# segeschecho/OpenEKFMonoSLAM

Measured on AMD Instinct MI355X. Metric: EKF updates/s (frames/s) at N features, higher is better.
Workload: dtype f32 storage; i8 MFMA with exact i32 sums (downdate) + f64 (B, S, state)

## Files before the change

include/ekf_test_hooks.h:

```cpp
#ifndef EKF_TEST_HOOKS_H
#define EKF_TEST_HOOKS_H

#include "ekf_engine.h"

#ifdef __cplusplus
extern "C" {
#endif

int ekf_debug_stall_next_sweep(EkfEngine *e);
int ekf_debug_stall_sweep_after(EkfEngine *e, int skip);
int ekf_debug_plane0_pieces(EkfEngine *e, int *nonzero, int *total);
int ekf_debug_dense_products(EkfEngine *e, int on);

#ifdef __cplusplus
}
#endif
#endif
```

openekfmonoslam_amd/csrc/engine.cpp:

```cpp
#include "engine.h"
#include "../../include/ekf_test_hooks.h"

#include <cmath>
#include <cstdio>
#include <algorithm>
#include <atomic>
#include <cstdlib>
#include <chrono>
#include <cstring>
#include <mutex>
#include <new>

#include <dlfcn.h>
#include <rccl/rccl.h>

using namespace ekf;

namespace ekf {
void launch_partition(EkfEngine *e, const EkfMatch *src, int M, const uint8_t *flags, EkfMatch *dst1, EkfMatch *dst0,
                      int *cnt1, bool map_update = false, const uint8_t *d_kdesc = nullptr, int *d_idx0 = nullptr,
                      int publish_seq = 0, bool rescue = false);
void launch_outlier_idx(EkfEngine *e, const EkfMatch *src, int M, int *idx);
}

// ... 1336 lines not shown
            e->pu_log.emplace_back(e->pu_m[i], ms);
        }
        (void)hipEventDestroy(e->pu_events[i].first);
        (void)hipEventDestroy(e->pu_events[i].second);
    }
    e->pu_events.clear();
    e->pu_work.clear();
    e->pu_m.clear();
    for (size_t i = 0; i < e->sw_events.size(); ++i) {
        float ms = 0.f;
        if (hipEventElapsedTime(&ms, e->sw_events[i].first, e->sw_events[i].second) == hipSuccess) {
            const double m = std::abs(e->sw_m[i]);
            e->sweep_ms += ms;
            e->sweep_panels += ((long long)m + NB - 1) / NB;
            e->sweep_launches += i < e->sw_launch.size() ? e->sw_launch[i] : 0;
            e->sweep_updates += 1;
            e->sweep_flops_f64 += m * m * m / 3.0;
            if (e->sw_m[i] > 0) e->sweep_flops_b += m * m * (double)e->n;
        }
        (void)hipEventDestroy(e->sw_events[i].first);
        (void)hipEventDestroy(e->sw_events[i].second);
    }
    e->sw_events.clear();
    e->sw_launch.clear();
    e->sw_m.clear();
}

struct StageTimer {
    EkfEngine *e;
    std::vector<hipEvent_t> evs;
    explicit StageTimer(EkfEngine *eng) : e(eng) {}
    ~StageTimer()
    {
        for (auto ev : evs) (void)hipEventDestroy(ev);
    }
    void mark()
    {
        if (!e->timing) return;
        hipEvent_t ev;
        if (hipEventCreate(&ev) != hipSuccess) return;
        (void)hipEventRecord(ev, e->stream);
        evs.push_back(ev);
    }
    void finish()
    {
        if (!e->timing || evs.size() < 7) return;
        (void)hipStreamSynchronize(e->stream);
        double *dst[6] = {&e->times.prediction_ms, &e->times.matching_ms, &e->times.ransac_ms,
                          &e->times.update_li_ms,  &e->times.rescue_ms,   &e->times.update_hi_ms};
        for (int i = 0; i < 6; ++i) {
            float ms = 0.f;
            if (hipEventElapsedTime(&ms, evs[i], evs[i + 1]) == hipSuccess) *dst[i] += ms;
        }
        for (auto ev : evs) (void)hipEventDestroy(ev);
        evs.clear();
        e->times.steps += 1;
        harvest_pu_events(e);
    }
};

static int match_ncc_dev(EkfEngine *e, int *n_matches);

static int detect_step_keypoints(EkfEngine *e);

static int step_dev(EkfEngine *e, const EkfKeypoint *d_kps, const uint8_t *d_desc, int n_kp, EkfStepInfo *info,
                    bool use_ncc = false, bool detect = false)
{
    const bool dev_counts = !use_ncc && !detect && !e->img.valid && !e->keep_step_preds && e->shard_world == 1;
    const bool lean = e->shard_world > 1;
    int *cnt = e->d.counts;
    EkfStepInfo li;
    std::memset(&li, 0, sizeof(li));
    int status = EKF_OK, rc;
    const int retries0 = e->sweep_retries;
    if (!dev_counts && e->err_unread) {
        if ((rc = read_counts(e))) return rc;
        if ((rc = recover_failed_update(e, &status))) return rc;
    }
    bool restarted = false;
restart:
    StageTimer tm(e);
    tm.mark();
    int np = 0;
    if (dev_counts) {
        const bool deferred = launch_predict_with_features(e, e->N);
        launch_hp_rows(e, e->d.plist, e->N, true, cnt + CNT_NPRED, deferred);
    } else {
        launch_predict(e);
        if ((rc = predict_measurements_dev(e, nullptr, e->N, &np, true, lean))) return rc;
    }
    tm.mark();
    int M = 0;
    if (dev_counts) {
        launch_match(e, d_kps, d_desc, e->N, n_kp, cnt + CNT_NPRED, true);
    } else {
        if (detect && (rc = detect_step_keypoints(e))) return rc;
        if (lean) rc = match_sharded_dev(e, use_ncc, d_kps, d_desc, n_kp, &M);
        else rc = use_ncc ? match_ncc_dev(e, &M) : match_dev(e, d_kps, d_desc, n_kp, &M, detect ? cnt + CNT_KP_FOUND : nullptr);
        if (rc) return rc;
    }
    tm.mark();
    if (dev_counts) {
        const int batch = e->cfg.ransac_batch;
        const int seq_r = next_publish_seq(e);
        launch_ransac_batch(e, e->N, 0, batch, cnt + CNT_NMATCH, seq_r);
        if ((rc = wait_counts(e, seq_r))) return rc;
        if (e->h_counts[CNT_ERR] && !restarted) {
            if ((rc = recover_failed_update(e, &status))) return rc;
            restarted = true;
            goto restart;
        }
        np = e->n_pred = e->h_counts[CNT_NPRED];
        M = e->h_counts[CNT_NMATCH];
        for (int h0 = batch, nb = batch * RANSAC_WIDE_FACTOR; !e->h_counts[CNT_RS_DONE] && h0 < M; h0 += nb) {
            launch_ransac_batch(e, M, h0, nb);
            if ((rc = read_counts(e))) return rc;
        }
    } else if (M > 0 && (rc = ransac_dev(e, M, lean))) {
        return rc;
    }
    li.n_predicted = np;
    li.n_matches = M;
    int ni = 0, no = 0;
    if (M > 0) {
        li.n_hypotheses = e->h_counts[CNT_RS_NEXT];
        ni = e->h_counts[CNT_RS_BEST];
        no = M - ni;
        launch_partition(e, e->d.matches, M, e->d.best_flags, e->d.msel, e->d.mout, nullptr, true, d_desc, e->d.work_idx);
    }
    li.n_inliers = ni;
    li.n_outliers = no;
    tm.mark();
    if ((rc = update_dev(e, ni, true, lean))) return rc;
    tm.mark();
    int nr = 0;
    if (no > 0) {
        int nop = 0;
        for (int attempt = 0; attempt < 2; ++attempt) {
            if (dev_counts) {
                launch_predict_features(e, e->d.work_idx, no, false);
                launch_hp_rows(e, e->d.plist_sub, no, false, cnt + CNT_NPRED_SUB);
                const int seq_p = next_publish_seq(e);
                launch_partition(e, e->d.mout, no, e->d.mask, e->d.msel, nullptr, cnt + CNT_NRESC, true, d_desc, nullptr, seq_p, true);
                rc = wait_counts(e, seq_p);
            } else {
                rc = predict_measurements_dev(e, e->d.work_idx, no, &nop, false, lean);
            }
            if (rc) return rc;
            if (!e->h_counts[CNT_ERR]) break;
            if ((rc = recover_failed_update(e, &status))) return rc;
        }
        if (dev_counts) {
            nr = e->h_counts[CNT_NRESC];
        } else if (nop > 0) {
            launch_rescue(e, e->d.mout, no);
            launch_partition(e, e->d.mout, no, e->d.mask, e->d.msel, nullptr, cnt + CNT_NRESC, true, d_desc);
            if ((rc = read_counts(e))) return rc;
            nr = e->h_counts[CNT_NRESC];
        }
    }
    li.n_rescued = nr;
    tm.mark();
    if ((rc = update_dev(e, nr, true, lean))) return rc;
    tm.mark();
    if (dev_counts && e->async_errors) {
        e->err_unread = true;
    } else {
        if ((rc = read_counts(e))) return rc;
        if (detect) {
            e->step_kp_detected = e->h_counts[CNT_KP_FOUND];
            e->step_kp_kept = std::min(e->step_kp_detected, e->kcap);
        }
        if ((rc = recover_failed_update(e, &status))) return rc;
    }
    tm.finish();
    li.status = status;
    li.n_sweep_retries = e->sweep_retries - retries0;
    if (info) *info = li;
    return status;
}

int ekf_set_async_errors(EkfEngine *e, int on)
{
    if (!e) return EKF_ERR_INVALID_ARG;
    e->async_errors = on != 0;
    return EKF_OK;
}

// ... 446 lines not shown
        launch_ncc_pyramid_on(e, e->stream2, e->img.px2, e->img.seq + (size_t)(frame + 1) * frame_bytes, e->img.seq_stride,
                              e->img.seq_channels);
        HIPCHK(hipEventRecord(e->ev_prefetch, e->stream2));
        e->img.prefetched = frame + 1;
    }
    return EKF_OK;
}

int ekf_select_staged_image(EkfEngine *e, int frame)
{
    if (!e) return EKF_ERR_INVALID_ARG;
    HIPCHK(hipSetDevice(e->device));
    int rc = staged_pyramid(e, frame);
    return rc ? rc : check_async(e);
}

int ekf_step_staged_image(EkfEngine *e, int frame, EkfStepInfo *info)
{
    if (!e) return EKF_ERR_INVALID_ARG;
    HIPCHK(hipSetDevice(e->device));
    int rc = staged_pyramid(e, frame);
    if (rc) return rc;
    return step_image_dev(e, info);
}

int ekf_timing_enable(EkfEngine *e, int on)
{
    if (!e) return EKF_ERR_INVALID_ARG;
    e->timing = on != 0;
    return EKF_OK;
}

int ekf_timing_reset(EkfEngine *e)
{
    if (!e) return EKF_ERR_INVALID_ARG;
    (void)hipStreamSynchronize(e->stream);
    harvest_pu_events(e);
    e->pu_log.clear();
    std::memset(&e->times, 0, sizeof(e->times));
    e->sweep_ms = e->sweep_flops_f64 = e->sweep_flops_b = 0.0;
    e->sweep_panels = e->sweep_updates = e->sweep_launches = 0;
    e->slice_ms = 0.0;
    return EKF_OK;
}

int ekf_timing_get(EkfEngine *e, EkfStageTimes *out)
{
    if (!e || !out) return EKF_ERR_INVALID_ARG;
    (void)hipStreamSynchronize(e->stream);
    harvest_pu_events(e);
    *out = e->times;
    return EKF_OK;
}

int ekf_timing_sweep(EkfEngine *e, double *kernel_ms, int64_t *panels, int64_t *updates, double *flops_fp64, double *flops_b)
{
    if (!e) return EKF_ERR_INVALID_ARG;
    (void)hipStreamSynchronize(e->stream);
    harvest_pu_events(e);
    if (kernel_ms) *kernel_ms = e->sweep_ms;
    if (panels) *panels = e->sweep_panels;
    if (updates) *updates = e->sweep_updates;
    if (flops_fp64) *flops_fp64 = e->sweep_flops_f64;
    if (flops_b) *flops_b = e->sweep_flops_b;
    return EKF_OK;
}

int ekf_get_sweep_retries(const EkfEngine *e) { return e ? e->sweep_retries : 0; }

int ekf_debug_stall_next_sweep(EkfEngine *e)
{
    if (!e) return EKF_ERR_INVALID_ARG;
    e->ps_fault = 1;
    return EKF_OK;
}

int ekf_debug_dense_products(EkfEngine *e, int on)
{
    if (!e) return EKF_ERR_INVALID_ARG;
    e->px_dense = on != 0;
    return EKF_OK;
}

int ekf_debug_plane0_pieces(EkfEngine *e, int *nonzero, int *total)
{
    if (!e || !nonzero || !total || !e->d.Bz) return EKF_ERR_INVALID_ARG;
    HIPCHK(hipSetDevice(e->device));
    HIPCHK(hipStreamSynchronize(e->stream));
    const int cbs = (e->n + 31) / 32, groups = (2 * e->last_update_M + 15) / 16;
    std::vector<uint8_t> row((size_t)e->bz_stride);
    int nz = 0;
    for (int c = 0; c < cbs; ++c) {
        HIPCHK(hipMemcpy(row.data(), e->d.Bz + (size_t)c * e->bz_stride, (size_t)groups, hipMemcpyDeviceToHost));
        for (int k = 0; k < groups; ++k) nz += row[k] ? 1 : 0;
    }
    *nonzero = nz;
    *total = cbs * groups;
    return EKF_OK;
}

int ekf_debug_stall_sweep_after(EkfEngine *e, int skip)
{
    if (!e || skip < 0) return EKF_ERR_INVALID_ARG;
    e->ps_fault = skip + 1;
    return EKF_OK;
}

int ekf_round_covariance_to_f32(EkfEngine *e)
{
    if (!e) return EKF_ERR_INVALID_ARG;
    if (e->f32) return EKF_ERR_INVALID_ARG;
    HIPCHK(hipSetDevice(e->device));
    launch_round_P_f32(e);
    return EKF_OK;
}

int ekf_timing_sweep_launches(EkfEngine *e, int64_t *launches, double *slice_ms)
{
    if (!e) return EKF_ERR_INVALID_ARG;
    (void)hipStreamSynchronize(e->stream);
    harvest_pu_events(e);
    if (launches) *launches = e->sweep_launches;
    if (slice_ms) *slice_ms = e->slice_ms;
    return EKF_OK;
}

int ekf_timing_p_update_launches(EkfEngine *e, int capacity, int32_t *m_rows, float *ms, int *count)
{
    if (!e || !count) return EKF_ERR_INVALID_ARG;
    (void)hipStreamSynchronize(e->stream);
    harvest_pu_events(e);
    *count = (int)e->pu_log.size();
    for (int i = 0; i < *count && i < capacity; ++i) {
        if (m_rows) m_rows[i] = e->pu_log[i].first;
        if (ms) ms[i] = e->pu_log[i].second;
    }
    return EKF_OK;
}

}
```

openekfmonoslam_amd/csrc/engine.h:

```cpp
#pragma once
#include <hip/hip_runtime.h>

#include <atomic>
#include <cstdint>
#include <map>
#include <memory>
#include <mutex>
#include <string>
#include <vector>

#include "../../include/ekf_engine.h"
#include "device_math.h"

namespace ekf {

constexpr int NB = 32;
constexpr int LD_ALIGN = 128;
constexpr int B_SWEEP_MAX = 2048;
constexpr int DX_SPLIT = 16;
constexpr int RANSAC_WIDE_FACTOR = 8;
#ifndef PX_S_VALUE
#define PX_S_VALUE 5
#endif
constexpr int PX_S = PX_S_VALUE;
constexpr int PX_MAX_ROWS = ((1 << 17) / PX_S) / 32 * 32;

inline int round_up(int v, int a) { return (v + a - 1) / a * a; }

constexpr int SHARD_BASE = 128;
struct RowMap {
    int r0, r1, base;
};
__host__ __device__ inline int local_row(const RowMap &m, int i) { return i < 13 ? i : m.base + (i - m.r0); }
__host__ __device__ inline bool owns_row(const RowMap &m, int i) { return i < 13 || (i >= m.r0 && i < m.r1); }

enum {
    CNT_NPRED = 0,
    CNT_NPRED_SUB,
    CNT_NMATCH,
    CNT_ERR,
    CNT_RS_BEST,
    CNT_RS_BESTH,
    CNT_RS_NHYP,
    CNT_RS_NEXT,
    CNT_RS_DONE,
    CNT_NRESC,
    CNT_KP_FOUND,
    CNT_AUX1,
    CNT_SHARD0,
    CNT_COUNT = 32
};
constexpr int MAX_SHARD_WORLD = 16;

enum { ST_X = 0, ST_R = 13, ST_F = 32, ST_GQG = 32 + 169, ST_JN = 32 + 338, ST_COUNT = 32 + 338 + 16 };

struct DeviceArrays {
    double *state = nullptr;
    double *feat_pos = nullptr;
    int *feat_type = nullptr;
    int *feat_covpos = nullptr;
    uint8_t *feat_desc = nullptr;
    unsigned *feat_times_predicted = nullptr;
    unsigned *feat_times_matched = nullptr;
    void *P = nullptr;
    void *P2 = nullptr;
    double *mm_scratch = nullptr;
    int *mm_index = nullptr;
    EkfMapPoint *map_points = nullptr;
    int *pred_vis = nullptr;
    int *pred_vis_full = nullptr;
    EkfPrediction *step_preds = nullptr;
    double *pred_uv = nullptr;
    int *pred_vis2 = nullptr;
    double *pred_uv2 = nullptr;
    double *pred_S = nullptr;
    double *Hs = nullptr;
    double *Hf = nullptr;
    void *HP = nullptr;
    int *work_idx = nullptr;
    int *work_flag = nullptr;
    int *plist = nullptr;
    int *plist_sub = nullptr;
    int *counts = nullptr;
    int *shard_feat = nullptr;
    EkfKeypoint *kps = nullptr;
    uint8_t *kdesc = nullptr;
    int *mt_valid = nullptr;
    int *mt_kp = nullptr;
    float *mt_dist = nullptr;
    EkfKeypoint *mt_xy = nullptr;
    uint8_t *tmpl = nullptr;
    double *gates = nullptr;
    unsigned long long *kp_rowmask = nullptr;
    EkfKeypoint *det_kps = nullptr;
    uint8_t *det_desc = nullptr;
    int *det_centres = nullptr;
    long long *cell_resp = nullptr;
    int *cell_xy = nullptr;
    EkfMatch *matches = nullptr;
    EkfMatch *msel = nullptr;
    EkfMatch *mout = nullptr;
    EkfPrediction *preds_out = nullptr;
// ... 141 lines not shown
    bool px_dense = false;
    int px_scale_shift = 0;
    int lq_nbk = 0;
    int bstage_rows = 0;
    std::vector<std::pair<hipEvent_t, hipEvent_t>> px_events;
    hipEvent_t px_mid = nullptr;
    int pu_slots = 0;
    int pu_parity = 0;
    hipStream_t stream = nullptr;
    hipStream_t stream2 = nullptr;
    hipEvent_t ev_main = nullptr, ev_prefetch = nullptr;
    ekf::DeviceArrays d;
    ekf::Frames frames;
    ekf::Image img;
    std::string err;
    bool timing = false;
    EkfStageTimes times{};
    hipEvent_t ev[4] = {nullptr, nullptr, nullptr, nullptr};
    std::vector<std::pair<hipEvent_t, hipEvent_t>> pu_events;
    std::vector<double> pu_work;
    std::vector<int> pu_m;
    std::vector<std::pair<int, float>> pu_log;
    std::vector<std::pair<hipEvent_t, hipEvent_t>> sw_events;
    std::vector<int> sw_m;
    std::vector<int> sw_launch;
    double sweep_ms = 0.0, sweep_flops_f64 = 0.0, sweep_flops_b = 0.0;
    long long sweep_panels = 0, sweep_updates = 0, sweep_launches = 0;
    double slice_ms = 0.0;
    std::vector<int> h_counts;
    int *h_mirror = nullptr, *d_mirror = nullptr;
    int mirror_seq = 0;
    std::vector<int> h_type, h_covpos;
};

namespace ekf {

struct XtyArgs {
    const void *X; int ldx; long long xb;
    const void *Y; int ldy; long long yb;
    void *C; int ldc; long long cb;
    void *Ct; int ldct; long long ctb;
    float *Ctf;
    int M, N, K;
    int row0_first, row0_stride, m_lim;
    int tri;
    int tiles_i, tiles_j;
    int tj0;
    int n_split;
    double alpha;
};
void launch_xty(EkfEngine *e, const XtyArgs &a, int batch, bool f32, hipStream_t stream);

#ifdef __HIPCC__
__device__ __forceinline__ bool filter_frozen(const int *counts) { return counts != nullptr && counts[CNT_ERR] != 0; }
#endif

#ifdef __HIPCC__
__device__ __forceinline__ int block_exclusive_scan_1024(int c, int *wtot , int *total)
{
    const int lane = threadIdx.x & 63, wv = threadIdx.x >> 6;
    int x = c;
#pragma unroll
    for (int o = 1; o < 64; o <<= 1) {
        const int y = __shfl_up(x, o, 64);
        if (lane >= o) x += y;
    }
    if (lane == 63) wtot[wv] = x;
    __syncthreads();
    int base = 0, tot = 0;
#pragma unroll
    for (int w = 0; w < 16; ++w) {
        const int t = wtot[w];
        base += w < wv ? t : 0;
        tot += t;
    }
    *total = tot;
    return base + x - c;
}
#endif

void launch_predict(EkfEngine *e);
bool launch_predict_features(EkfEngine *e, const int *d_idx, int count, bool state_only, bool defer_compact = false);
bool launch_predict_with_features(EkfEngine *e, int count);
void launch_hp_rows(EkfEngine *e, const int *d_list, int n_list, bool count_predicted = false, const int *d_count = nullptr, bool from_flags = false);
void launch_match(EkfEngine *e, const EkfKeypoint *kps, const uint8_t *kdesc, int n_pred, int n_kp, const int *d_npred = nullptr,
                  bool with_ransac_init = false, const int *d_nkp = nullptr);
void launch_match_index(EkfEngine *e, int M, const int *d_M = nullptr);
void launch_shard_bounds(EkfEngine *e, const EkfMatch *list, int count);
void launch_shard_bounds_idx(EkfEngine *e, const int *list, const int *d_count);
void launch_match_slots(EkfEngine *e, const EkfKeypoint *kps, const uint8_t *kdesc, int n_kp, int s_lo, int s_hi);
void launch_match_ncc_slots(EkfEngine *e, int s_lo, int s_hi);
void launch_match_compact(EkfEngine *e, const EkfKeypoint *kps, int n_pred);
void launch_match_compact_slots(EkfEngine *e, int n_pred, const EkfKeypoint *d_slot_xy);
void launch_ransac_hyp(EkfEngine *e, int M, int h0, int batch, const int *d_M, int h_lo, int h_hi);
void launch_ransac_select(EkfEngine *e, int M, int h0, int batch, const int *d_M, int publish_seq);
void launch_ransac_batch(EkfEngine *e, int M, int h0, int batch, const int *d_M = nullptr, int publish_seq = 0);
void launch_ransac_init(EkfEngine *e, int M);
void launch_update(EkfEngine *e, int M, bool update_cov);
void launch_p_update_exact(EkfEngine *e, int m, bool use_bc, bool exps_ready = false, bool planes_ready = false);
void launch_round_P_f32(EkfEngine *e);
void launch_diag_extract(EkfEngine *e, float *diag);
void launch_planes_move(EkfEngine *e, bool pack, int m_k, int c_lo, int c_hi, int skip_lo, int skip_hi);
void launch_dx_planes(EkfEngine *e, int m_k);
void launch_slice_columns(EkfEngine *e, int m, int c_lo, int c_hi);
void launch_b_gemm_planes(EkfEngine *e, int m, int c_lo, int c_hi);
void launch_rescue(EkfEngine *e, const EkfMatch *matches, int M);
void launch_state_only_predict(EkfEngine *e, EkfPrediction *d_out);
void launch_add_features(EkfEngine *e, const double *d_uv, int count, double *d_Jpo, double *d_Jhr);
void launch_compact_P(EkfEngine *e, int n_new, const int *d_new2old);
void launch_linearity(EkfEngine *e, double *d_out);
void launch_convert(EkfEngine *e, int fi, int pos, double *d_J, double *d_T3);
void launch_map_points(EkfEngine *e, EkfMapPoint *d_out);
void launch_ncc_pyramid(EkfEngine *e, const uint8_t *d_raw, int stride, int channels);
void launch_ncc_pyramid_on(EkfEngine *e, hipStream_t stream, uint8_t *const px[3], const uint8_t *d_raw, int stride, int channels);
void launch_ncc_capture(EkfEngine *e, const int *d_idx, const double *d_uv, int count);
void launch_match_ncc(EkfEngine *e, int n_pred);
void launch_gate_snapshot(EkfEngine *e, int n_pred);
void launch_detect_cells(EkfEngine *e, int n_gates, int cells_x, int cells_y, long long *d_resp, int *d_xy);
void launch_kp_detect(EkfEngine *e, long long thr, bool masked, unsigned long long *rowmask, EkfKeypoint *out, int cap, int *d_found);
size_t kp_rowmask_words(int w, int h);
void launch_brief(EkfEngine *e, const EkfKeypoint *kps, const int *centres, int n, const int *d_n, uint8_t *desc);
void launch_publish_counts(EkfEngine *e, int *d_mirror, int seq);
__device__ __forceinline__ void publish_counts_block(const int *counts, int *mirror, int seq)
{
    __syncthreads();
    const int t = threadIdx.x;
    if (t < 64) {
        if (t < CNT_COUNT) __hip_atomic_store(&mirror[t], counts[t], __ATOMIC_RELAXED, __HIP_MEMORY_SCOPE_SYSTEM);
        __threadfence_system();
        __builtin_amdgcn_wave_barrier();
        if (t == 0) {
            __threadfence_system();
            __hip_atomic_store(&mirror[CNT_COUNT], seq, __ATOMIC_RELEASE, __HIP_MEMORY_SCOPE_SYSTEM);
        }
    }
}
void launch_pack_predictions(EkfEngine *e, const int *d_list, int n, EkfPrediction *d_out);

}
```

openekfmonoslam_amd/csrc/kernels_predict.hip:

```cpp
#include "engine.h"

namespace ekf {

__device__ void predict_prepare_serial(double *st, double *sG);

__global__ void __launch_bounds__(256) k_predict_prepare(double *st, ParD par, const int *counts)
{
    __shared__ double sG[13 * 6];
    if (filter_frozen(counts)) return;
    const double dt = 1.0;
    const double ln = par.linearAccelSD * par.linearAccelSD * dt * dt;
    const double an = par.angularAccelSD * par.angularAccelSD * dt * dt;
    if (blockIdx.x != 0) return;
    if (threadIdx.x == 0) predict_prepare_serial(st, sG);
    __syncthreads();
    if (threadIdx.x < 169) {
        const int i = threadIdx.x / 13, j = threadIdx.x % 13;
        double s = 0.0;
        for (int k = 0; k < 6; ++k) s += (sG[i * 6 + k] * (k < 3 ? ln : an)) * sG[j * 6 + k];
        st[ST_GQG + i * 13 + j] = s;
    }
}

__device__ void predict_prepare_serial(double *st, double *sG)
// ... 183 lines not shown
    if (ok) list[pos] = fi;
    if (threadIdx.x == 0) *out_count = total;
}

template <int BLOCK>
__global__ void __launch_bounds__(BLOCK)
k_predict_features(const double *st, CamD cam, const double *feat_pos, const int *feat_type, const int *idx,
                   int count, int *flag, int *vis, double *uv_tab, double *Hs_tab, double *Hf_tab, int *vis_full, int *list, int *out_count)
{
    predict_features_body<BLOCK>((int)blockIdx.x, st, cam, feat_pos, feat_type, idx, count, flag, vis, uv_tab, Hs_tab, Hf_tab, vis_full, list, out_count);
}

template <typename T>
__global__ void __launch_bounds__(256)
k_predict_cov_features(int nb_cov, T *P, int ld, int n, RowMap rm, const double *st, CamD cam, const double *feat_pos, const int *feat_type,
                       int count, int *flag, int *vis, double *uv_tab, double *Hs_tab, double *Hf_tab, int *vis_full, int *list, int *out_count,
                       const int *counts)
{
    if ((int)blockIdx.x < nb_cov) {
        if (filter_frozen(counts)) return;
        predict_cov_body<T>((int)blockIdx.x, P, ld, n, st, rm);
    } else predict_features_body<256>((int)blockIdx.x - nb_cov, st, cam, feat_pos, feat_type, nullptr, count, flag, vis, uv_tab, Hs_tab, Hf_tab,
                                    vis_full, list, out_count);
}

bool launch_predict_with_features(EkfEngine *e, int count)
{
    if (count <= 0) {
        launch_predict(e);
        return launch_predict_features(e, nullptr, count, false, true);
    }
    k_predict_prepare<<<1, 256, 0, e->stream>>>(e->d.state, e->par, e->d.counts);
    const int nb_cov = 1 + (e->n > 13 ? (e->n - 13 + 255) / 256 : 0);
    const int nb_f = (count + 255) / 256;
    const bool one = count <= 256;
    int *list = one ? e->d.plist : nullptr, *cnt = one ? e->d.counts + CNT_NPRED : nullptr;
#define PCF_ARGS e->ldP, e->n, e->rm, e->d.state, e->cam, e->d.feat_pos, e->d.feat_type, count, e->d.work_flag, e->d.pred_vis, e->d.pred_uv, e->d.Hs, \
                 e->d.Hf, e->d.pred_vis_full, list, cnt, e->d.counts
    if (e->f32) k_predict_cov_features<float><<<nb_cov + nb_f, 256, 0, e->stream>>>(nb_cov, (float *)e->d.P, PCF_ARGS);
    else k_predict_cov_features<double><<<nb_cov + nb_f, 256, 0, e->stream>>>(nb_cov, (double *)e->d.P, PCF_ARGS);
#undef PCF_ARGS
    return !one;
}

__global__ void __launch_bounds__(1024) k_compact(const int *flag, const int *idx, int count, int *list, int *out_count)
{
    __shared__ int wtot[16];
    const int tid = threadIdx.x;
    const int per = (count + 1023) / 1024;
    const int b = tid * per, e = min(count, b + per);
    int c = 0;
    for (int i = b; i < e; ++i) c += flag[i] ? 1 : 0;
    int total;
    int pos = block_exclusive_scan_1024(c, wtot, &total);
    for (int i = b; i < e; ++i)
        if (flag[i]) list[pos++] = idx ? idx[i] : i;
    if (tid == 1023) *out_count = total;
}

bool launch_predict_features(EkfEngine *e, const int *d_idx, int count, bool state_only, bool defer_compact)
{
    const bool sub = state_only || d_idx != nullptr;
    if (count <= 0) {
        (void)hipMemsetAsync(e->d.counts + (sub ? CNT_NPRED_SUB : CNT_NPRED), 0, sizeof(int), e->stream);
        return false;
    }
    int *list = sub ? e->d.plist_sub : e->d.plist, *cnt = e->d.counts + (sub ? CNT_NPRED_SUB : CNT_NPRED);
#define PF_ARGS(L_, C_) e->d.state, e->cam, e->d.feat_pos, e->d.feat_type, d_idx, count, e->d.work_flag, state_only ? e->d.pred_vis2 : e->d.pred_vis, \
                        state_only ? e->d.pred_uv2 : e->d.pred_uv, state_only ? nullptr : e->d.Hs, state_only ? nullptr : e->d.Hf,                      \
                        sub ? nullptr : e->d.pred_vis_full, L_, C_
    if (count <= 256) {
        k_predict_features<256><<<1, 256, 0, e->stream>>>(PF_ARGS(list, cnt));
        return false;
    }
    const int nb = (count + 255) / 256;
    k_predict_features<256><<<nb, 256, 0, e->stream>>>(PF_ARGS(nullptr, nullptr));
#undef PF_ARGS
    if (defer_compact && !sub && !d_idx) return true;
    k_compact<<<1, 1024, 0, e->stream>>>(e->d.work_flag, d_idx, count, sub ? e->d.plist_sub : e->d.plist,
                                         e->d.counts + (sub ? CNT_NPRED_SUB : CNT_NPRED));
    return false;
}

template <typename T, typename TO>
__global__ void __launch_bounds__(256)
k_hp_rows(const T *P, int ld, int n, const int *list, const int *feat_type, const int *feat_covpos,
          const double *Hs_tab, const double *Hf_tab, TO *HP, double *S_tab, RowMap rm, double *HPc, unsigned *times_predicted,
          const int *d_count, const int *flag, int n_items, int *list_out, int *count_out, const int *counts)
{
    const int tid = threadIdx.x;
    if (flag) {
        if ((int)blockIdx.x == n_items) {
            if (blockIdx.y != 0) return;
            __shared__ int wtot[16];
            if (tid < 16) wtot[tid] = 0;
            __syncthreads();
            const int per = (n_items + 255) / 256;
            const int b = tid * per, e = min(n_items, b + per);
            int c = 0;
            for (int i = b; i < e; ++i) c += flag[i] ? 1 : 0;
            int total;
            int pos = block_exclusive_scan_1024(c, wtot, &total);
            for (int i = b; i < e; ++i)
                if (flag[i]) list_out[pos++] = i;
            if (tid == 0) *count_out = total;
            return;
        }
        if (!flag[blockIdx.x]) return;
    } else if (d_count && (int)blockIdx.x >= *d_count) return;
    __shared__ double sH[26];
    __shared__ double sHP[2][13];
    const int fi = flag ? (int)blockIdx.x : list[blockIdx.x];
    const int d = feat_dim(feat_type[fi]);
    const int pos = feat_covpos[fi];
    const bool first = blockIdx.y == 0;
    if (times_predicted && tid == 0 && first && !filter_frozen(counts)) times_predicted[fi]++;
    if (!owns_row(rm, pos)) return;
    const T *Pf = P + (size_t)local_row(rm, pos) * ld;
    if (tid < 14) sH[tid] = Hs_tab[14 * fi + tid];
    else if (tid < 26) sH[tid] = Hf_tab[12 * fi + tid - 14];
    double pcol[13];
    int jcol = -1;
    if (first && tid >= 64 && tid < 64 + 7 + d) {
        jcol = tid - 64 < 7 ? tid - 64 : pos + (tid - 64 - 7);
#pragma unroll
        for (int a = 0; a < 6; ++a) pcol[a] = a < d ? (double)Pf[(size_t)a * ld + jcol] : 0.0;
#pragma unroll
        for (int a = 0; a < 7; ++a) pcol[6 + a] = (double)P[(size_t)a * ld + jcol];
    }
    __syncthreads();
    if (jcol >= 0) {
        double a0 = 0.0, a1 = 0.0, b0 = 0.0, b1 = 0.0;
#pragma unroll
        for (int a = 0; a < 6; ++a)
            if (a < d) {
                a0 += sH[14 + a] * pcol[a];
                a1 += sH[20 + a] * pcol[a];
            }
#pragma unroll
        for (int a = 0; a < 7; ++a) {
            b0 += sH[a] * pcol[6 + a];
            b1 += sH[7 + a] * pcol[6 + a];
        }
        sHP[0][tid - 64] = a0 + b0;
        sHP[1][tid - 64] = a1 + b1;
    }
    TO *o0 = HP + (size_t)(2 * fi) * ld;
    TO *o1 = o0 + ld;
    constexpr int VW = 16 / sizeof(T);
    typedef T vec_t __attribute__((ext_vector_type(VW)));
    const int jb = ((int)blockIdx.y * 256 + tid) * VW;
    if (jb < n) {
        vec_t pf[6], pc[7];
#pragma unroll
        for (int a = 0; a < 6; ++a)
            if (a < d) pf[a] = *(const vec_t *)(Pf + (size_t)a * ld + jb);
#pragma unroll
        for (int a = 0; a < 7; ++a) pc[a] = *(const vec_t *)(P + (size_t)a * ld + jb);
        typedef TO ovec_t __attribute__((ext_vector_type(VW)));
        ovec_t r0, r1;
#pragma unroll
        for (int v = 0; v < VW; ++v) {
            const int j = jb + v;
            double a0 = 0.0, a1 = 0.0;
#pragma unroll
            for (int a = 0; a < 6; ++a)
                if (a < d) {
                    const double p = (double)pf[a][v];
                    a0 += sH[14 + a] * p;
                    a1 += sH[20 + a] * p;
                }
            double b0 = 0.0, b1 = 0.0;
#pragma unroll
            for (int a = 0; a < 7; ++a) {
                const double p = (double)pc[a][v];
                b0 += sH[a] * p;
                b1 += sH[7 + a] * p;
            }
            a0 += b0;
            a1 += b1;
            r0[v] = (TO)a0;
            r1[v] = (TO)a1;
            if (j < 13) {
                HPc[(size_t)(2 * fi) * 16 + j] = a0;
                HPc[(size_t)(2 * fi + 1) * 16 + j] = a1;
            }
        }
        if (jb + VW <= n) {
            *(ovec_t *)(o0 + jb) = r0;
            *(ovec_t *)(o1 + jb) = r1;
        } else {
#pragma unroll
            for (int v = 0; v < VW; ++v)
                if (jb + v < n) { o0[jb + v] = r0[v]; o1[jb + v] = r1[v]; }
        }
    }
    if (!first) return;
    __syncthreads();
    if (tid < 4) {
        const int r = tid >> 1, c = tid & 1;
        double s1 = 0.0, s2 = 0.0;
        for (int a = 0; a < 7; ++a) s1 += sHP[r][a] * sH[c * 7 + a];
        for (int a = 0; a < d; ++a) s2 += sHP[r][7 + a] * sH[14 + c * 6 + a];
        S_tab[4 * fi + tid] = s1 + s2 + (r == c ? 1.0 : 0.0);
    }
}

void launch_hp_rows(EkfEngine *e, const int *d_list, int n_list, bool count_predicted, const int *d_count, bool from_flags)
{
    unsigned *tp = count_predicted ? e->d.feat_times_predicted : nullptr;
    if (n_list <= 0) return;
    const int chunks_f = (e->n + 256 * 4 - 1) / (256 * 4), chunks_d = (e->n + 256 * 2 - 1) / (256 * 2);
    const int *flag = from_flags ? e->d.work_flag : nullptr;
    int *lo = from_flags ? e->d.plist : nullptr, *co = from_flags ? e->d.counts + CNT_NPRED : nullptr;
    const int gx = n_list + (from_flags ? 1 : 0);
    if (e->exact && e->f32)
        k_hp_rows<float, double><<<dim3(gx, chunks_f), 256, 0, e->stream>>>((const float *)e->d.P, e->ldP, e->n, d_list, e->d.feat_type,
                                                        e->d.feat_covpos, e->d.Hs, e->d.Hf, (double *)e->d.HP,
                                                        e->d.pred_S, e->rm, e->d.HPc, tp, d_count, flag, n_list, lo, co, e->d.counts);
    else if (e->f32)
        k_hp_rows<float, float><<<dim3(gx, chunks_f), 256, 0, e->stream>>>((const float *)e->d.P, e->ldP, e->n, d_list, e->d.feat_type,
                                                        e->d.feat_covpos, e->d.Hs, e->d.Hf, (float *)e->d.HP,
                                                        e->d.pred_S, e->rm, e->d.HPc, tp, d_count, flag, n_list, lo, co, e->d.counts);
    else
        k_hp_rows<double, double><<<dim3(gx, chunks_d), 256, 0, e->stream>>>((const double *)e->d.P, e->ldP, e->n, d_list,
                                                         e->d.feat_type, e->d.feat_covpos, e->d.Hs, e->d.Hf,
                                                         (double *)e->d.HP, e->d.pred_S, e->rm, e->d.HPc, tp, d_count, flag, n_list, lo, co, e->d.counts);
}

__global__ void __launch_bounds__(256)
k_pack_predictions(const int *list, const int *count, const double *uv_tab, const double *S_tab, EkfPrediction *out,
                   int with_S)
{
    const int k = blockIdx.x * 256 + threadIdx.x;
    if (k >= *count) return;
    const int fi = list[k];
    EkfPrediction p;
    p.featureIndex = fi;
    p._pad = 0;
    p.imagePos[0] = uv_tab[2 * fi];
    p.imagePos[1] = uv_tab[2 * fi + 1];
    for (int i = 0; i < 4; ++i) p.covarianceMatrix[i] = with_S ? S_tab[4 * fi + i] : 0.0;
    out[k] = p;
}

__global__ void __launch_bounds__(256)
k_pack_predictions_n(const int *list, int n, const double *uv_tab, const double *S_tab, EkfPrediction *out)
{
    const int k = blockIdx.x * 256 + threadIdx.x;
    if (k >= n) return;
    const int fi = list[k];
    EkfPrediction p;
    p.featureIndex = fi;
    p._pad = 0;
    p.imagePos[0] = uv_tab[2 * fi];
    p.imagePos[1] = uv_tab[2 * fi + 1];
    for (int i = 0; i < 4; ++i) p.covarianceMatrix[i] = S_tab[4 * fi + i];
    out[k] = p;
}

void launch_pack_predictions(EkfEngine *e, const int *d_list, int n, EkfPrediction *d_out)
{
    if (n > 0) k_pack_predictions_n<<<(n + 255) / 256, 256, 0, e->stream>>>(d_list, n, e->d.pred_uv, e->d.pred_S, d_out);
}

void launch_state_only_predict(EkfEngine *e, EkfPrediction *d_out)
{
    launch_predict_features(e, nullptr, e->N, true);
    if (e->N > 0)
        k_pack_predictions<<<(e->N + 255) / 256, 256, 0, e->stream>>>(e->d.plist_sub, e->d.counts + CNT_NPRED_SUB,
                                                                      e->d.pred_uv2, e->d.pred_S, d_out, 0);
}

}
```

openekfmonoslam_amd/engine.py:

```python
import ctypes as C
import os

import numpy as np

from .ekftypes import (DESC_BYTES, KEYPOINT_DTYPE, MAP_POINT_DTYPE, MATCH_DTYPE, PREDICTION_DTYPE, STATUS_NAMES, EkfCamera,
                       EkfMapPoint, EkfParams, EkfStepInfo)

_HERE = os.path.dirname(os.path.abspath(__file__))
LIB_PATH = os.path.join(_HERE, "libekf_engine.so")
PRECISION_F64, PRECISION_F32, PRECISION_F32_EXACT, PRECISION_F64_EXACT, PRECISION_AUTO = 0, 1, 2, 3, 4
IMAGE_MATCHER_NCC, IMAGE_MATCHER_KEYPOINTS = 0, 1


class EkfEngineConfig(C.Structure):
    _fields_ = [
        ("cam", EkfCamera),
        ("par", EkfParams),
        ("max_features", C.c_int32),
        ("max_keypoints", C.c_int32),
        ("precision", C.c_int32),
        ("device", C.c_int32),
        ("ransac_batch", C.c_int32),
        ("flags", C.c_int32),
    ]
# ... 12 lines not shown
        ("p_update_flops", C.c_double),
        ("p_update_bytes", C.c_double),
        ("steps", C.c_int64),
    ]


_vp, _i = C.c_void_p, C.c_int
ABI = {
    "ekf_engine_create": (_i, [C.POINTER(EkfEngineConfig), C.POINTER(_vp)]),
    "ekf_engine_destroy": (None, [_vp]),
    "ekf_last_error": (C.c_char_p, [_vp]),
    "ekf_abi_version": (_i, []),
    "ekf_device_count": (_i, []),
    "ekf_set_state": (_i, [_vp, _vp, _i, _vp, _vp, _vp, _vp]),
    "ekf_get_state": (_i, [_vp, _vp, _vp, _vp]),
    "ekf_get_map_features": (_i, [_vp, _vp, _vp, _vp]),
    "ekf_reset": (_i, [_vp]),
    "ekf_add_features": (_i, [_vp, _vp, _vp, _i]),
    "ekf_remove_features": (_i, [_vp, _vp, _i]),
    "ekf_remove_bad_features": (_i, [_vp, C.POINTER(_i)]),
    "ekf_convert_inverse_depth_to_depth": (_i, [_vp, C.POINTER(_i)]),
    "ekf_get_feature_layout": (_i, [_vp, _vp, _vp]),
    "ekf_keep_step_predictions": (_i, [_vp, _i]),
    "ekf_get_step_predictions": (_i, [_vp, _vp, C.POINTER(_i)]),
    "ekf_get_camera_covariance": (_i, [_vp, _vp]),
    "ekf_get_map_points": (_i, [_vp, C.POINTER(EkfMapPoint), _i, C.POINTER(_i)]),
    "ekf_get_unseen_features": (_i, [_vp, _vp, C.POINTER(_i)]),
    "ekf_state_dim": (_i, [_vp]),
    "ekf_descriptor_bytes": (_i, [_vp]),
    "ekf_num_features": (_i, [_vp]),
    "ekf_predict": (_i, [_vp]),
    "ekf_predict_measurements": (_i, [_vp, _vp, _i, _vp, C.POINTER(_i), _vp, _vp]),
    "ekf_predict_measurement_state": (_i, [_vp, _vp, C.POINTER(_i)]),
    "ekf_match": (_i, [_vp, _vp, _vp, _i, _vp, C.POINTER(_i)]),
    "ekf_ransac": (_i, [_vp, _vp, _i, _vp, C.POINTER(_i)]),
    "ekf_update": (_i, [_vp, _vp, _i]),
    "ekf_update_only_state": (_i, [_vp, _vp, _i]),
    "ekf_rescue": (_i, [_vp, _vp, _i, _vp]),
    "ekf_step": (_i, [_vp, _vp, _vp, _i, C.POINTER(EkfStepInfo)]),
    "ekf_frames_upload": (_i, [_vp, _i, _vp, _vp, _vp]),
    "ekf_step_frame": (_i, [_vp, _i, C.POINTER(EkfStepInfo)]),
    "ekf_set_async_errors": (_i, [_vp, _i]),
    "ekf_set_update_path": (_i, [_vp, _i]),
    "ekf_set_sweep_mode": (_i, [_vp, _i]),
    "ekf_get_precision": (_i, [_vp]),
    "ekf_image_upload": (_i, [_vp, _vp, _i, _i, _i, _i]),
    "ekf_get_image_level": (_i, [_vp, _i, _vp, C.POINTER(_i), C.POINTER(_i)]),
    "ekf_capture_templates": (_i, [_vp, _vp, _vp, _i]),
    "ekf_match_ncc": (_i, [_vp, _vp, C.POINTER(_i)]),
    "ekf_step_image": (_i, [_vp, _vp, _i, _i, _i, _i, C.POINTER(EkfStepInfo)]),
    "ekf_detect_new_features": (_i, [_vp, _i, _i, C.c_double, C.c_double, _vp, C.POINTER(_i)]),
    "ekf_images_upload": (_i, [_vp, _i, _vp, _i, _i, _i, _i]),
    "ekf_select_staged_image": (_i, [_vp, _i]),
    "ekf_step_staged_image": (_i, [_vp, _i, C.POINTER(EkfStepInfo)]),
    "ekf_set_image_matcher": (_i, [_vp, _i, C.c_double]),
    "ekf_detect_keypoints": (_i, [_vp, C.c_double, _i, _vp, _vp, _i, C.POINTER(_i)]),
    "ekf_describe": (_i, [_vp, _vp, _i, _vp]),
    "ekf_get_step_keypoints": (_i, [_vp, C.POINTER(_i), C.POINTER(_i)]),
    "ekf_timing_enable": (_i, [_vp, _i]),
    "ekf_timing_reset": (_i, [_vp]),
    "ekf_timing_get": (_i, [_vp, C.POINTER(EkfStageTimes)]),
    "ekf_synchronize": (_i, [_vp]),
    "ekf_timing_p_update_launches": (_i, [_vp, _i, _vp, _vp, C.POINTER(_i)]),
    "ekf_timing_sweep": (_i, [_vp, C.POINTER(C.c_double), C.POINTER(C.c_int64), C.POINTER(C.c_int64), C.POINTER(C.c_double),
                              C.POINTER(C.c_double)]),
    "ekf_timing_sweep_launches": (_i, [_vp, C.POINTER(C.c_int64), C.POINTER(C.c_double)]),
    "ekf_round_covariance_to_f32": (_i, [_vp]),
    "ekf_get_sweep_retries": (_i, [_vp]),
    "ekf_shard_rows": (_i, [_i, _i, _i, C.POINTER(_i), C.POINTER(_i)]),
    "ekf_engine_create_sharded": (_i, [C.POINTER(EkfEngineConfig), _i, _i, C.POINTER(_vp)]),
    "ekf_set_exchange": (_i, [_vp, _vp, _vp]),
    "ekf_comm_unique_id": (_i, [_vp]),
    "ekf_comm_init": (_i, [_vp, _vp]),
    "ekf_shard_info": (_i, [_vp, C.POINTER(_i), C.POINTER(_i), C.POINTER(_i), C.POINTER(_i)]),
    "ekf_shard_counters": (_i, [_vp, C.POINTER(C.c_int64), C.POINTER(C.c_int32), C.POINTER(C.c_int32)]),
    "ekf_device_copy": (_i, [_vp, _vp, _vp, C.c_size_t]),
}

TEST_HOOKS = {
    "ekf_debug_stall_next_sweep": (_i, [_vp]),
    "ekf_debug_stall_sweep_after": (_i, [_vp, _i]),
    "ekf_debug_plane0_pieces": (_i, [_vp, C.POINTER(_i), C.POINTER(_i)]),
    "ekf_debug_dense_products": (_i, [_vp, _i]),
}

EXCHANGE_FN = C.CFUNCTYPE(_i, _vp, _i, _vp, C.c_size_t, C.POINTER(C.c_int32), _i, _i)
XCHG_HP, XCHG_PRED_S = 0, 1

_lib = None


def load_library():
    global _lib
    if _lib is not None:
        return _lib
    if not os.path.exists(LIB_PATH):
        raise RuntimeError(
            f"{LIB_PATH} is missing: build it with `python -m openekfmonoslam_amd.build` (hipcc, gfx950). "
            "There is no CPU fallback."
        )
    try:
        import torch
    except Exception:
        pass
    override = os.environ.get("EKF_ENGINE_LIB")
    L = C.CDLL(os.path.abspath(override) if override else LIB_PATH)
    for name, (rt, at) in list(ABI.items()) + list(TEST_HOOKS.items()):
        if override and not hasattr(L, name):
            continue
        fn = getattr(L, name)
        fn.restype = rt
        fn.argtypes = at
    _lib = L
    return L


class EkfError(RuntimeError):
    def __init__(self, code, msg=""):
        super().__init__(f"{STATUS_NAMES.get(code, code)}: {msg}")
        self.code = code


def _p(a):
    return a.ctypes.data_as(C.c_void_p) if a is not None else None


def shard_rows(n_features, world, rank):
    lo, hi = _i(0), _i(0)
    rc = load_library().ekf_shard_rows(n_features, world, rank, C.byref(lo), C.byref(hi))
    if rc:
        raise EkfError(rc)
    return lo.value, hi.value


def comm_unique_id():
    buf = np.zeros(128, dtype=np.uint8)
    rc = load_library().ekf_comm_unique_id(_p(buf))
    if rc:
        raise EkfError(rc, "ekf_comm_unique_id (librccl.so.1 not loadable?)")
    return buf


class EkfEngine:

    def __init__(self, cam, par, max_features, max_keypoints=0, precision=PRECISION_F64, device=-1, ransac_batch=0,
                 shard=None, descriptor_cols_f32=0):
        self.L = load_library()
        cfg = EkfEngineConfig()
        cfg.cam, cfg.par = cam, par
        cfg.max_features, cfg.max_keypoints = int(max_features), int(max_keypoints)
        cfg.precision, cfg.device, cfg.ransac_batch = int(precision), int(device), int(ransac_batch)
        cfg.flags = (1 | (int(descriptor_cols_f32) << 8)) if descriptor_cols_f32 else 0
        h = _vp()
        if shard is None:
            rc = self.L.ekf_engine_create(C.byref(cfg), C.byref(h))
        else:
            rc = self.L.ekf_engine_create_sharded(C.byref(cfg), int(shard[0]), int(shard[1]), C.byref(h))
        self._xchg_ref = None
        if rc:
            raise EkfError(rc, "ekf_engine_create failed (no MI355X visible?)")
        self.h = h
        self.cap = int(max_features)
        self.precision = int(self.L.ekf_get_precision(self.h))
        self.desc_bytes = self.L.ekf_descriptor_bytes(self.h)
        self.desc_dtype = np.float32 if descriptor_cols_f32 else np.uint8

# ... 27 lines not shown
        self._chk(self.L.ekf_shard_info(self.h, C.byref(r), C.byref(w), C.byref(lo), C.byref(hi)))
        return r.value, w.value, lo.value, hi.value

    def shard_counters(self):
        b, c0, c1 = C.c_int64(0), C.c_int32(0), C.c_int32(0)
        self._chk(self.L.ekf_shard_counters(self.h, C.byref(b), C.byref(c0), C.byref(c1)))
        return b.value, c0.value, c1.value

    def device_copy(self, dst, src, nbytes):
        self._chk(self.L.ekf_device_copy(self.h, _vp(dst), _vp(src), nbytes))

    def close(self):
        if getattr(self, "h", None):
            self.L.ekf_engine_destroy(self.h)
            self.h = None

    def __del__(self):
        self.close()

    def _chk(self, rc, allow=()):
        if rc and rc not in allow:
            raise EkfError(rc, (self.L.ekf_last_error(self.h) or b"").decode())
        return rc

    @property
    def n(self):
        return self.L.ekf_state_dim(self.h)

    @property
    def N(self):
        return self.L.ekf_num_features(self.h)

    def set_state(self, x13, feature_pos, feature_type, desc, P):
        x13 = np.ascontiguousarray(x13, dtype=np.float64)
        fp = np.ascontiguousarray(feature_pos, dtype=np.float64).reshape(-1, 6)
        ft = None if feature_type is None else np.ascontiguousarray(feature_type, dtype=np.int32)
        d = self._desc(desc)
        Pm = None if P is None else np.ascontiguousarray(P, dtype=np.float64)
        self._chk(self.L.ekf_set_state(self.h, _p(x13), len(fp), _p(fp), _p(ft), _p(d), _p(Pm)))

    def get_state(self, want_P=True, P_out=None):
        x = np.zeros(13)
        fp = np.zeros((max(self.N, 1), 6))
        P = P_out if P_out is not None else (np.zeros((self.n, self.n)) if want_P else None)
        self._chk(self.L.ekf_get_state(self.h, _p(x), _p(fp), _p(P)))
        return x, fp[: self.N], P

    def camera_covariance(self):
        P = np.zeros((13, 13))
        self._chk(self.L.ekf_get_camera_covariance(self.h, _p(P)))
        return P

    def map_points(self):
        buf = (EkfMapPoint * max(self.N, 1))()
        n = _i(0)
        self._chk(self.L.ekf_get_map_points(self.h, buf, len(buf), C.byref(n)))
        return np.frombuffer(buf, dtype=MAP_POINT_DTYPE)[: n.value]

    def unseen_features(self):
        idx = np.zeros(max(self.N, 1), dtype=np.int32)
        n = C.c_int(0)
        self._chk(self.L.ekf_get_unseen_features(self.h, _p(idx), C.byref(n)))
        return idx[: n.value].copy()

    def set_async_errors(self, on=True):
        if hasattr(self.L, "ekf_set_async_errors"):
            self._chk(self.L.ekf_set_async_errors(self.h, 1 if on else 0))

    @property
    def sweep_retries(self):
        return int(self.L.ekf_get_sweep_retries(self.h))

    def stall_sweep(self, skip=0):
        self._chk(self.L.ekf_debug_stall_sweep_after(self.h, int(skip)))

    def plane0_pieces(self):
        a, b = _i(0), _i(0)
        self._chk(self.L.ekf_debug_plane0_pieces(self.h, C.byref(a), C.byref(b)))
        return a.value, b.value

    def dense_products(self, on=True):
        self._chk(self.L.ekf_debug_dense_products(self.h, 1 if on else 0))

    def set_update_path(self, path):
        self._chk(self.L.ekf_set_update_path(self.h, int(path)))

    def set_sweep_mode(self, mode):
        self._chk(self.L.ekf_set_sweep_mode(self.h, int(mode)))

    def keep_step_predictions(self, on=True):
        self._chk(self.L.ekf_keep_step_predictions(self.h, 1 if on else 0))

    def step_predictions(self):
        from .ekftypes import PREDICTION_DTYPE

        n = C.c_int(0)
        self._chk(self.L.ekf_get_step_predictions(self.h, None, C.byref(n)))
        out = np.zeros(max(n.value, 1), dtype=PREDICTION_DTYPE)
        self._chk(self.L.ekf_get_step_predictions(self.h, _p(out), C.byref(n)))
        return out[: n.value].copy()

    def reset(self):
        self._chk(self.L.ekf_reset(self.h))

    def add_features(self, uv, desc=None):
        uv = np.ascontiguousarray(uv, dtype=np.float64).reshape(-1, 2)
        d = self._desc(desc)
        self._chk(self.L.ekf_add_features(self.h, _p(uv), _p(d), len(uv)))

    def remove_features(self, idx):
        idx = np.ascontiguousarray(idx, dtype=np.int32)
        self._chk(self.L.ekf_remove_features(self.h, _p(idx), len(idx)))

    def remove_bad_features(self):
        k = _i(0)
        self._chk(self.L.ekf_remove_bad_features(self.h, C.byref(k)))
        return k.value

    def convert_inverse_depth_to_depth(self):
        k = _i(-1)
        self._chk(self.L.ekf_convert_inverse_depth_to_depth(self.h, C.byref(k)))
        return k.value

    def feature_layout(self):
        t = np.zeros(max(self.N, 1), dtype=np.int32)
        c = np.zeros(max(self.N, 1), dtype=np.int32)
        self._chk(self.L.ekf_get_feature_layout(self.h, _p(t), _p(c)))
        return t[: self.N], c[: self.N]

    def get_map_features(self):
        N = max(self.N, 1)
        d = np.zeros((N, self.desc_bytes), dtype=np.uint8)
        tp = np.zeros(N, dtype=np.uint32)
        tm = np.zeros(N, dtype=np.uint32)
        self._chk(self.L.ekf_get_map_features(self.h, _p(d), _p(tp), _p(tm)))
        return d[: self.N].view(self.desc_dtype), tp[: self.N], tm[: self.N]

    def predict(self):
        self._chk(self.L.ekf_predict(self.h))

    def predict_measurements(self, feat_idx=None):
        idx = None if feat_idx is None else np.ascontiguousarray(feat_idx, dtype=np.int32)
        cnt = 0 if idx is None else len(idx)
        cap = self.N if idx is None else max(cnt, 1)
        preds = np.zeros(max(cap, 1), dtype=PREDICTION_DTYPE)
        Hs = np.zeros((max(cap, 1), 2, 13))
        Hf = np.zeros((max(cap, 1), 2, 6))
        k = _i(0)
        self._chk(self.L.ekf_predict_measurements(self.h, _p(idx), cnt, _p(preds), C.byref(k), _p(Hs), _p(Hf)))
        return preds[: k.value].copy(), Hs[: k.value].copy(), Hf[: k.value].copy()

    def predict_measurement_state(self):
        preds = np.zeros(max(self.N, 1), dtype=PREDICTION_DTYPE)
        k = _i(0)
        self._chk(self.L.ekf_predict_measurement_state(self.h, _p(preds), C.byref(k)))
        return preds[: k.value].copy()

    def match(self, kps, desc):
        kps = np.ascontiguousarray(kps, dtype=KEYPOINT_DTYPE)
        desc = self._desc(desc)
        out = np.zeros(max(self.N, 1), dtype=MATCH_DTYPE)
        k = _i(0)
        self._chk(self.L.ekf_match(self.h, _p(kps), _p(desc), len(kps), _p(out), C.byref(k)))
        return out[: k.value].copy()

    def ransac(self, matches):
# ... 159 lines not shown
```

Before: 1202.

## Compute full HP rows only for matched features, S-only pass for all predictions

For large feature counts, the predict stage now runs an S-only variant of the HP kernel over all predicted features. The full H*P rows are computed afterwards only for matched features, in two launches placed around the first RANSAC batch. This avoids streaming covariance rows for predicted features that never match. The cost is extra kernel launches, a dependency on the match list layout, and the assumption that downstream code reads HP rows by match index. A debug hook that poisons HP buffers is added for testing.

```diff
diff --git a/include/ekf_test_hooks.h b/include/ekf_test_hooks.h
--- a/include/ekf_test_hooks.h
+++ b/include/ekf_test_hooks.h
@@ -11,6 +11,7 @@
 int ekf_debug_stall_sweep_after(EkfEngine *e, int skip);
 int ekf_debug_plane0_pieces(EkfEngine *e, int *nonzero, int *total);
 int ekf_debug_dense_products(EkfEngine *e, int on);
+int ekf_debug_poison_hp(EkfEngine *e);
 
 #ifdef __cplusplus
 }
diff --git a/openekfmonoslam_amd/csrc/engine.cpp b/openekfmonoslam_amd/csrc/engine.cpp
--- a/openekfmonoslam_amd/csrc/engine.cpp
+++ b/openekfmonoslam_amd/csrc/engine.cpp
@@ -1442,9 +1442,11 @@
     StageTimer tm(e);
     tm.mark();
     int np = 0;
+    const bool hp_split = dev_counts && e->N >= HP_SPLIT_MIN_N;
     if (dev_counts) {
         const bool deferred = launch_predict_with_features(e, e->N);
-        launch_hp_rows(e, e->d.plist, e->N, true, cnt + CNT_NPRED, deferred);
+        if (hp_split) launch_hp_s_only(e, e->N, cnt + CNT_NPRED, deferred);
+        else launch_hp_rows(e, e->d.plist, e->N, true, cnt + CNT_NPRED, deferred);
     } else {
         launch_predict(e);
         if ((rc = predict_measurements_dev(e, nullptr, e->N, &np, true, lean))) return rc;
@@ -1463,7 +1465,9 @@
     if (dev_counts) {
         const int batch = e->cfg.ransac_batch;
         const int seq_r = next_publish_seq(e);
+        if (hp_split) launch_hp_rows_matched(e, 0, std::min(batch, e->N), cnt + CNT_NMATCH);
         launch_ransac_batch(e, e->N, 0, batch, cnt + CNT_NMATCH, seq_r);
+        if (hp_split) launch_hp_rows_matched(e, batch, e->N, cnt + CNT_NMATCH);
         if ((rc = wait_counts(e, seq_r))) return rc;
         if (e->h_counts[CNT_ERR] && !restarted) {
             if ((rc = recover_failed_update(e, &status))) return rc;
@@ -2076,6 +2080,16 @@
     return EKF_OK;
 }
 
+int ekf_debug_poison_hp(EkfEngine *e)
+{
+    if (!e || !e->d.HP || !e->d.HPc) return EKF_ERR_INVALID_ARG;
+    HIPCHK(hipSetDevice(e->device));
+    const size_t wb = e->exact ? 8 : (e->f32 ? 4 : 8);
+    HIPCHK(hipMemsetAsync(e->d.HP, 0xFF, (size_t)e->mcap * e->ldP * wb, e->stream));
+    HIPCHK(hipMemsetAsync(e->d.HPc, 0xFF, (size_t)e->mcap * 16 * sizeof(double), e->stream));
+    return EKF_OK;
+}
+
 int ekf_debug_plane0_pieces(EkfEngine *e, int *nonzero, int *total)
 {
     if (!e || !nonzero || !total || !e->d.Bz) return EKF_ERR_INVALID_ARG;
diff --git a/openekfmonoslam_amd/csrc/engine.h b/openekfmonoslam_amd/csrc/engine.h
--- a/openekfmonoslam_amd/csrc/engine.h
+++ b/openekfmonoslam_amd/csrc/engine.h
@@ -18,6 +18,9 @@
 constexpr int LD_ALIGN = 128;
 constexpr int B_SWEEP_MAX = 2048;
 constexpr int DX_SPLIT = 16;
+#ifndef HP_SPLIT_MIN_N
+#define HP_SPLIT_MIN_N 257
+#endif
 constexpr int RANSAC_WIDE_FACTOR = 8;
 #ifndef PX_S_VALUE
 #define PX_S_VALUE 5
@@ -325,7 +328,11 @@
 void launch_predict(EkfEngine *e);
 bool launch_predict_features(EkfEngine *e, const int *d_idx, int count, bool state_only, bool defer_compact = false);
 bool launch_predict_with_features(EkfEngine *e, int count);
-void launch_hp_rows(EkfEngine *e, const int *d_list, int n_list, bool count_predicted = false, const int *d_count = nullptr, bool from_flags = false);
+enum { HP_FULL = 0, HP_S_ONLY = 1, HP_ROWS = 2 };
+void launch_hp_rows(EkfEngine *e, const int *d_list, int n_list, bool count_predicted = false, const int *d_count = nullptr, bool from_flags = false,
+                    int mode = HP_FULL, const EkfMatch *d_matches = nullptr, int k0 = 0, int k1 = 0);
+void launch_hp_s_only(EkfEngine *e, int n_list, const int *d_count, bool from_flags);
+void launch_hp_rows_matched(EkfEngine *e, int k0, int k1, const int *d_M);
 void launch_match(EkfEngine *e, const EkfKeypoint *kps, const uint8_t *kdesc, int n_pred, int n_kp, const int *d_npred = nullptr,
                   bool with_ransac_init = false, const int *d_nkp = nullptr);
 void launch_match_index(EkfEngine *e, int M, const int *d_M = nullptr);
diff --git a/openekfmonoslam_amd/csrc/kernels_predict.hip b/openekfmonoslam_amd/csrc/kernels_predict.hip
--- a/openekfmonoslam_amd/csrc/kernels_predict.hip
+++ b/openekfmonoslam_amd/csrc/kernels_predict.hip
@@ -289,14 +289,17 @@
     return false;
 }
 
-template <typename T, typename TO>
+template <typename T, typename TO, int MODE>
 __global__ void __launch_bounds__(256)
 k_hp_rows(const T *P, int ld, int n, const int *list, const int *feat_type, const int *feat_covpos,
           const double *Hs_tab, const double *Hf_tab, TO *HP, double *S_tab, RowMap rm, double *HPc, unsigned *times_predicted,
-          const int *d_count, const int *flag, int n_items, int *list_out, int *count_out, const int *counts)
+          const int *d_count, const int *flag, int n_items, int *list_out, int *count_out, const int *counts,
+          const EkfMatch *mlist, int k0, int k1)
 {
     const int tid = threadIdx.x;
-    if (flag) {
+    if (MODE == HP_ROWS) {
+        if (k0 + (int)blockIdx.x >= min(k1, *d_count)) return;
+    } else if (flag) {
         if ((int)blockIdx.x == n_items) {
             if (blockIdx.y != 0) return;
             __shared__ int wtot[16];
@@ -317,11 +320,11 @@
     } else if (d_count && (int)blockIdx.x >= *d_count) return;
     __shared__ double sH[26];
     __shared__ double sHP[2][13];
-    const int fi = flag ? (int)blockIdx.x : list[blockIdx.x];
+    const int fi = MODE == HP_ROWS ? mlist[k0 + (int)blockIdx.x].featureIndex : (flag ? (int)blockIdx.x : list[blockIdx.x]);
     const int d = feat_dim(feat_type[fi]);
     const int pos = feat_covpos[fi];
-    const bool first = blockIdx.y == 0;
-    if (times_predicted && tid == 0 && first && !filter_frozen(counts)) times_predicted[fi]++;
+    const bool first = MODE != HP_ROWS && blockIdx.y == 0;
+    if (MODE != HP_ROWS && times_predicted && tid == 0 && first && !filter_frozen(counts)) times_predicted[fi]++;
     if (!owns_row(rm, pos)) return;
     const T *Pf = P + (size_t)local_row(rm, pos) * ld;
     if (tid < 14) sH[tid] = Hs_tab[14 * fi + tid];
@@ -357,7 +360,7 @@
     constexpr int VW = 16 / sizeof(T);
     typedef T vec_t __attribute__((ext_vector_type(VW)));
     const int jb = ((int)blockIdx.y * 256 + tid) * VW;
-    if (jb < n) {
+    if (MODE != HP_S_ONLY && jb < n) {
         vec_t pf[6], pc[7];
 #pragma unroll
         for (int a = 0; a < 6; ++a)
@@ -413,26 +416,40 @@
     }
 }
 
-void launch_hp_rows(EkfEngine *e, const int *d_list, int n_list, bool count_predicted, const int *d_count, bool from_flags)
+void launch_hp_rows(EkfEngine *e, const int *d_list, int n_list, bool count_predicted, const int *d_count, bool from_flags, int mode,
+                    const EkfMatch *d_matches, int k0, int k1)
 {
     unsigned *tp = count_predicted ? e->d.feat_times_predicted : nullptr;
     if (n_list <= 0) return;
-    const int chunks_f = (e->n + 256 * 4 - 1) / (256 * 4), chunks_d = (e->n + 256 * 2 - 1) / (256 * 2);
+    const int chunks_f = mode == HP_S_ONLY ? 1 : (e->n + 256 * 4 - 1) / (256 * 4), chunks_d = mode == HP_S_ONLY ? 1 : (e->n + 256 * 2 - 1) / (256 * 2);
     const int *flag = from_flags ? e->d.work_flag : nullptr;
     int *lo = from_flags ? e->d.plist : nullptr, *co = from_flags ? e->d.counts + CNT_NPRED : nullptr;
     const int gx = n_list + (from_flags ? 1 : 0);
-    if (e->exact && e->f32)
-        k_hp_rows<float, double><<<dim3(gx, chunks_f), 256, 0, e->stream>>>((const float *)e->d.P, e->ldP, e->n, d_list, e->d.feat_type,
-                                                        e->d.feat_covpos, e->d.Hs, e->d.Hf, (double *)e->d.HP,
-                                                        e->d.pred_S, e->rm, e->d.HPc, tp, d_count, flag, n_list, lo, co, e->d.counts);
-    else if (e->f32)
-        k_hp_rows<float, float><<<dim3(gx, chunks_f), 256, 0, e->stream>>>((const float *)e->d.P, e->ldP, e->n, d_list, e->d.feat_type,
-                                                        e->d.feat_covpos, e->d.Hs, e->d.Hf, (float *)e->d.HP,
-                                                        e->d.pred_S, e->rm, e->d.HPc, tp, d_count, flag, n_list, lo, co, e->d.counts);
-    else
-        k_hp_rows<double, double><<<dim3(gx, chunks_d), 256, 0, e->stream>>>((const double *)e->d.P, e->ldP, e->n, d_list,
-                                                         e->d.feat_type, e->d.feat_covpos, e->d.Hs, e->d.Hf,
-                                                         (double *)e->d.HP, e->d.pred_S, e->rm, e->d.HPc, tp, d_count, flag, n_list, lo, co, e->d.counts);
+#define HP_LAUNCH(T_, TO_, CH_)                                                                                                                    \
+    do {                                                                                                                                           \
+        const dim3 grid(gx, CH_);                                                                                                                  \
+        if (mode == HP_S_ONLY) k_hp_rows<T_, TO_, HP_S_ONLY><<<grid, 256, 0, e->stream>>>(HP_ARGS(T_, TO_));                                       \
+        else if (mode == HP_ROWS) k_hp_rows<T_, TO_, HP_ROWS><<<grid, 256, 0, e->stream>>>(HP_ARGS(T_, TO_));                                      \
+        else k_hp_rows<T_, TO_, HP_FULL><<<grid, 256, 0, e->stream>>>(HP_ARGS(T_, TO_));                                                           \
+    } while (0)
+#define HP_ARGS(T_, TO_) (const T_ *)e->d.P, e->ldP, e->n, d_list, e->d.feat_type, e->d.feat_covpos, e->d.Hs, e->d.Hf, (TO_ *)e->d.HP, e->d.pred_S, e->rm, \
+                         e->d.HPc, tp, d_count, flag, n_list, lo, co, e->d.counts, d_matches, k0, k1
+    if (e->exact && e->f32) HP_LAUNCH(float, double, chunks_f);
+    else if (e->f32) HP_LAUNCH(float, float, chunks_f);
+    else HP_LAUNCH(double, double, chunks_d);
+#undef HP_ARGS
+#undef HP_LAUNCH
+}
+
+void launch_hp_s_only(EkfEngine *e, int n_list, const int *d_count, bool from_flags)
+{
+    launch_hp_rows(e, e->d.plist, n_list, true, d_count, from_flags, HP_S_ONLY);
+}
+
+void launch_hp_rows_matched(EkfEngine *e, int k0, int k1, const int *d_M)
+{
+    if (k1 <= k0) return;
+    launch_hp_rows(e, nullptr, k1 - k0, false, d_M, false, HP_ROWS, e->d.matches, k0, k1);
 }
 
 __global__ void __launch_bounds__(256)
diff --git a/openekfmonoslam_amd/engine.py b/openekfmonoslam_amd/engine.py
--- a/openekfmonoslam_amd/engine.py
+++ b/openekfmonoslam_amd/engine.py
@@ -118,6 +118,7 @@
     "ekf_debug_stall_sweep_after": (_i, [_vp, _i]),
     "ekf_debug_plane0_pieces": (_i, [_vp, C.POINTER(_i), C.POINTER(_i)]),
     "ekf_debug_dense_products": (_i, [_vp, _i]),
+    "ekf_debug_poison_hp": (_i, [_vp]),
 }
 
 EXCHANGE_FN = C.CFUNCTYPE(_i, _vp, _i, _vp, C.c_size_t, C.POINTER(C.c_int32), _i, _i)
@@ -311,6 +312,9 @@
     def dense_products(self, on=True):
         self._chk(self.L.ekf_debug_dense_products(self.h, 1 if on else 0))
 
+    def poison_hp(self):
+        self._chk(self.L.ekf_debug_poison_hp(self.h))
+
     def set_update_path(self, path):
         self._chk(self.L.ekf_set_update_path(self.h, int(path)))
 
```

After: 1223 (median of 6 runs). +1.7%, better.
